# ComparativeGenomicsToolkit/cactus

Hardware: NVIDIA H100
Metric: BAR POA DP Gcells/sec and ends/sec at 1/2/4/8 H100 vs reference CPU BAR (higher is better)
Workload: dtype int32

## Files before the change

### cactus_b200/csrc/poa_kernel.cu

```cuda
#include <cuda_runtime.h>
#include <stdint.h>
#include "poa_graph.cuh"
#include "poa_cta.cuh"
#include "poa_kernel.cuh"

namespace barb200 {

#define FULL 0xffffffffu

struct KShared {
    Graph g; RowTables rt; DpState d;
    int job, msa_len_s, abort_s;
    __align__(256) int smat[5 * 8];
    int wF[2][2][32];
    int wM[2][4][32];
    RowRec rec[2];
    RowInfo ring_info[2];
};

__device__ __forceinline__ int4 ld4cg(const int *p) { return __ldcg(reinterpret_cast<const int4 *>(p)); }
__device__ __forceinline__ void st4(int *p, int a, int b, int c, int d) {
    asm volatile("st.global.v4.s32 [%0], {%1, %2, %3, %4};" ::"l"(p), "r"(a), "r"(b), "r"(c), "r"(d) : "memory");
}
__device__ __forceinline__ void sts4(unsigned a, int x, int y, int z, int w) {
    asm volatile("st.shared.v4.s32 [%0], {%1, %2, %3, %4};" ::"r"(a), "r"(x), "r"(y), "r"(z), "r"(w) : "memory");
}
__device__ __forceinline__ int4 lds4(unsigned a) {
    int4 v;
    asm volatile("ld.shared.v4.s32 {%0, %1, %2, %3}, [%4];" : "=r"(v.x), "=r"(v.y), "=r"(v.z), "=r"(v.w) : "r"(a) : "memory");
    return v;
}
__device__ __forceinline__ int lds1(unsigned a) {
    int v;
    asm volatile("ld.shared.s32 %0, [%1];" : "=r"(v) : "r"(a) : "memory");
    return v;
}
__device__ __forceinline__ int lds_const(unsigned a) {
    int v;
    asm("ld.shared.s32 %0, [%1];" : "=r"(v) : "r"(a));
    return v;
}
__device__ __forceinline__ int max3(int a, int b, int c) { return max(max(a, b), c); }
__device__ __forceinline__ void cp_async16(void *smem, const void *gmem) {
    asm volatile("cp.async.cg.shared.global [%0], [%1], 16;" ::"r"((unsigned)__cvta_generic_to_shared(smem)), "l"(gmem) : "memory");
}
__device__ __forceinline__ void cp_async_wait_all() { asm volatile("cp.async.wait_all;" ::: "memory"); }
__device__ __forceinline__ void store_pad(int *tp, int64_t cs, int NEG) {
#pragma unroll
    for (int c = 0; c < TB / CHUNK; ++c) st4(tp + c * cs, c < CPT / CHUNK ? NEG : 0, c < CPT / CHUNK ? NEG : 0, c < CPT / CHUNK ? NEG : 0, c < CPT / CHUNK ? NEG : 0);
}


template <bool MASKED>
__device__ __forceinline__ void row_pass1(int (&H)[CPT], int (&E1)[CPT], int (&E2)[CPT], unsigned mbase, const uint32_t (&qo)[4],
                                          int j0, int beg, int end, int NEG, int e1, int e2, int &agg1, int &agg2) {
#pragma unroll
    for (int e = 0; e < CPT; ++e) {
        const int s = lds_const(__byte_perm(qo[e >> 2], mbase, 0x7650 | (e & 3)));
        int h = __vimax3_s32(H[e] + s, E1[e], E2[e]);
        if (MASKED) {
            const bool inb = (unsigned)(j0 + e - beg) <= (unsigned)(end - beg);
            h = inb ? h : NEG; E1[e] = inb ? E1[e] : NEG; E2[e] = inb ? E2[e] : NEG;
        }
        H[e] = h;
    }
    int a1 = H[CPT - 1], a2 = H[CPT - 1];
#pragma unroll
    for (int e = CPT - 2; e >= 0; --e) { a1 = __viaddmax_s32(a1, e1, H[e]); a2 = __viaddmax_s32(a2, e2, H[e]); }
    agg1 = max(agg1, a1 + j0 * e1); agg2 = max(agg2, a2 + j0 * e2);
}

template <bool ROW0>
__device__ __forceinline__ void pred_chunk(int (&H)[CPT], int (&E1)[CPT], int (&E2)[CPT], int oc, int4 h4, int4 d4, int NEG) {
    const int h[CHUNK] = {h4.x, h4.y, h4.z, h4.w}, dv[CHUNK] = {d4.x, d4.y, d4.z, d4.w};
#pragma unroll
    for (int u = 0; u < CHUNK; ++u) {
        const int e = oc * CHUNK + u;
        const int c1 = dv[u] & 0xffff, c2 = (int)((unsigned)dv[u] >> 16);
        if (e + 1 < CPT) H[e + 1] = max(H[e + 1], h[u]);
        E1[e] = max(E1[e], ROW0 && c1 == E_NEG16 ? NEG : h[u] - c1); E2[e] = max(E2[e], ROW0 && c2 == E_NEG16 ? NEG : h[u] - c2);
    }
}

template <int MODE, int RING_NT>
__device__ __forceinline__ void row_pass2(int (&H)[CPT], int (&E1)[CPT], int (&E2)[CPT], int F1, int F2, int j0, int beg, int end, int NEG,
                                          int e1, int e2, int oe1, int oe2, int *tp, int64_t cs, unsigned rs, int &tmax) {
#pragma unroll
    for (int oc = 0; oc < CPT / CHUNK; ++oc) {
        int dd[CHUNK];
#pragma unroll
        for (int u = 0; u < CHUNK; ++u) {
            const int e = oc * CHUNK + u, hp = H[e];
            int h = __vimax3_s32(hp, F1, F2);
            F1 = __viaddmax_s32(F1, -e1, hp - oe1); F2 = __viaddmax_s32(F2, -e2, hp - oe2);
            int x1 = __viaddmax_s32(E1[e], -e1, h - oe1);
            int x2 = __viaddmax_s32(E2[e], -e2, h - oe2);
            if (MODE == 1) {
                const bool inb = (unsigned)(j0 + e - beg) <= (unsigned)(end - beg);
                h = inb ? h : NEG; x1 = inb ? x1 : NEG; x2 = inb ? x2 : NEG;
            } else if (MODE == 2) {
                const bool inb = j0 + e <= end;
                h = inb ? h : NEG; x1 = inb ? x1 : NEG; x2 = inb ? x2 : NEG;
            }
            H[e] = h; E1[e] = x1; E2[e] = x2;
            dd[u] = __byte_perm(h - x1, h - x2, 0x5410);
            tmax = max(tmax, h);
        }
        st4(tp + oc * cs, H[oc * CHUNK], H[oc * CHUNK + 1], H[oc * CHUNK + 2], H[oc * CHUNK + 3]);
        st4(tp + (CPT / CHUNK + oc) * cs, dd[0], dd[1], dd[2], dd[3]);
        if (RING_NT) {
            sts4(rs + oc * RING_NT * 16, H[oc * CHUNK], H[oc * CHUNK + 1], H[oc * CHUNK + 2], H[oc * CHUNK + 3]);
            sts4(rs + (CPT / CHUNK + oc) * RING_NT * 16, dd[0], dd[1], dd[2], dd[3]);
        }
    }
}

template <bool MASKED>
__device__ __forceinline__ void row_argmax(const int (&H)[CPT], int v, int j0, int beg, int end, int &tl, int &tr) {
    unsigned m = 0;
#pragma unroll
    for (int e = 0; e < CPT; ++e) m |= H[e] == v ? 1u << e : 0u;
    if (MASKED) {
        const int lo = max(beg - j0, 0), hi = min(end - j0, CPT - 1);
        m &= (2u << hi) - (1u << lo);
    }
    if (m) { tl = j0 + __ffs(m) - 1; tr = j0 + 31 - __clz(m); }
}

template <int NT>
__device__ long long dp_sweep(KShared &S, const BatchArgs &A, const uint8_t *__restrict__ qg, int L, uint4 *qsm, unsigned ring) {
    constexpr int RING_NT = poa_ring_bytes(NT) ? NT : 0;
    constexpr unsigned SLOT = NT * TB * sizeof(int), RCS = NT * 16;
    const int tid = threadIdx.x, lane = tid & 31, warp = tid >> 5, nwarps = NT >> 5;
    const unsigned my_ring = ring + tid * 16;
    const PoaParams &P = A.P;
    uint8_t *const sb = A.slots + (int64_t)blockIdx.x * A.lay.slot_bytes;
    const RowRec *const rec_tab = reinterpret_cast<const RowRec *>(sb + A.lay.o_row_rec);
    const int *const pre_row = reinterpret_cast<const int *>(sb + A.lay.o_pre_row);
    RowInfo *const info = reinterpret_cast<RowInfo *>(sb + A.lay.o_row_info);
    int64_t *const row_off = reinterpret_cast<int64_t *>(sb + A.lay.o_row_off);
    int *const planes = A.planes + (int64_t)blockIdx.x * A.lay.plane_cap;
    const int64_t plane_cap = A.lay.plane_cap;
    const int node_n = S.g.node_n, R = node_n - 1;
    const int NEG = P.inf_min, e1 = P.e1, e2 = P.e2, oe1 = P.o1 + P.e1, oe2 = P.o2 + P.e2;
    const int w = P.wb + (int)(P.wf * L);
    const int pn_shift = reference_lane_count(P, L, node_n) == 16 ? 4 : 3;
    static_assert(CPT == 16, "shifts below assume 16 columns per thread");
    const int j0 = tid * CPT;

    uint32_t qo[4] = {0u, 0u, 0u, 0u};
#pragma unroll
    for (int e = 0; e < CPT; ++e) {
        const int j = j0 + e;
        const uint32_t c = (j >= 1 && j <= L) ? qg[j - 1] : 5u;
        qo[e >> 2] |= (4u * c) << ((e & 3) * 8);
    }
    qsm[tid] = make_uint4(qo[0], qo[1], qo[2], qo[3]);
    const unsigned smat_s = (unsigned)__cvta_generic_to_shared(S.smat);

    int H[CPT], E1[CPT], E2[CPT];
    bool prev_active;
    int prev_beg = 0, prev_end, prev_left = 0, prev_right = 0;
    int cur_blk = 0, cells = 0;

    {
        const int dd = L - rec_tab[0].rd;
        prev_end = min(L, max(0, dd) + w);
        const int nT = prev_end / CPT + 1, nTs = row_blocks(0, prev_end);
        if ((int64_t)nTs * TB > plane_cap) return -1;
        prev_active = tid < nT;
        int D[CPT];
#pragma unroll
        for (int e = 0; e < CPT; ++e) {
            const int j = j0 + e;
            if (j == 0) { H[e] = 0; E1[e] = -oe1; E2[e] = -oe2; D[e] = oe1 | (oe2 << 16); }
            else if (j <= prev_end) { H[e] = max(-P.o1 - e1 * j, -P.o2 - e2 * j); E1[e] = NEG; E2[e] = NEG; D[e] = E_NEG16 | (E_NEG16 << 16); }
            else { H[e] = E1[e] = E2[e] = NEG; D[e] = 0; }
        }
        if (tid < nTs) {
            int *tp = planes + chunk_index(nTs, tid, 0);
            const int64_t cs = chunk_index(nTs, 0, 1);
#pragma unroll
            for (int oc = 0; oc < CPT / CHUNK; ++oc) {
                st4(tp + oc * cs, H[oc * CHUNK], H[oc * CHUNK + 1], H[oc * CHUNK + 2], H[oc * CHUNK + 3]);
                st4(tp + (CPT / CHUNK + oc) * cs, D[oc * CHUNK], D[oc * CHUNK + 1], D[oc * CHUNK + 2], D[oc * CHUNK + 3]);
            }
        }
        if (RING_NT) {
#pragma unroll
            for (int oc = 0; oc < CPT / CHUNK; ++oc) {
                sts4(my_ring + oc * RCS, H[oc * CHUNK], H[oc * CHUNK + 1], H[oc * CHUNK + 2], H[oc * CHUNK + 3]);
                sts4(my_ring + (CPT / CHUNK + oc) * RCS, D[oc * CHUNK], D[oc * CHUNK + 1], D[oc * CHUNK + 2], D[oc * CHUNK + 3]);
            }
        }
        if (lane == 31) S.wM[0][3][warp] = H[CPT - 1];
        if (tid == 0) {
            RowInfo ri; ri.beg = 0; ri.end = prev_end; ri.left = 0; ri.right = 0; info[0] = ri; row_off[0] = 0;
            if (RING_NT) S.ring_info[0] = ri;
        }
        cur_blk = nTs; cells = prev_end + 1;
        if (tid == 0) { cp_async16(&S.rec[1], rec_tab + (R > 1 ? 1 : 0)); cp_async_wait_all(); }
    }
    __syncthreads();

    for (int r = 1; r < R; ++r) {
        const int par = r & 1;
        const RowRec rec = S.rec[par];
        if (tid == 0 && r + 1 < R) cp_async16(&S.rec[par ^ 1], rec_tab + r + 1);
        const int b = rec.base_npre & 0xff, npre = rec.base_npre >> 8;
        const int dd = L - rec.rd;
        int maxL = node_n, maxR = 0, min_pre_beg = 0x7fffffff;
        bool has_prev = false;
        if (npre == 1 && rec.pre0 == r - 1) {
            maxL = min(node_n, prev_left + 1); maxR = prev_right + 1; min_pre_beg = prev_beg; has_prev = true;
        } else {
#pragma unroll 1
            for (int k = 0; k < npre; ++k) {
                const int p = k == 0 ? rec.pre0 : pre_row[rec.pre_off + k];
                int pl, pr, pb;
                if (p == r - 1) { pl = prev_left; pr = prev_right; pb = prev_beg; has_prev = true; }
                else if (RING_NT && p == r - 2) { const RowInfo pi = S.ring_info[par]; pl = pi.left; pr = pi.right; pb = pi.beg; }
                else { const RowInfo pi = info[p]; pl = pi.left; pr = pi.right; pb = pi.beg; }
                maxL = min(maxL, pl + 1); maxR = max(maxR, pr + 1); min_pre_beg = min(min_pre_beg, pb);
            }
        }
        const bool only_prev = npre == 1 && has_prev;
        int beg = max(0, min(maxL, dd) - w);
        const int end = min(L, max(maxR, dd) + w);
        if ((beg >> pn_shift) < (min_pre_beg >> pn_shift)) beg = min_pre_beg;
        const int t0 = beg >> 4, nT = (end >> 4) - t0 + 1, tt = tid - t0;
        const int nTs = row_blocks(beg, end), tts = tid - row_t0(beg);
        if ((int64_t)(cur_blk + nTs) * TB > plane_cap) return -1;
        const bool active = tt >= 0 && tt < nT;
        const int wmode = __any_sync(FULL, active && j0 < beg) ? 1 : __any_sync(FULL, active && j0 + CPT - 1 > end) ? 2 : 0;
        const uint32_t qadd = 0x01010101u * (32u * b);

        int hl = __shfl_up_sync(FULL, prev_active ? H[CPT - 1] : NEG, 1);
        if (lane == 0) hl = warp > 0 ? S.wM[par ^ 1][3][warp - 1] : NEG;

        const int id1 = NEG + beg * e1 + P.o1, id2 = NEG + beg * e2 + P.o2;
        int agg1 = id1, agg2 = id2;
        if (active) {
            if (has_prev && prev_active) {
#pragma unroll
                for (int e = CPT - 1; e >= 1; --e) H[e] = H[e - 1];
                H[0] = hl;
            } else {
#pragma unroll
                for (int e = 0; e < CPT; ++e) { H[e] = NEG; E1[e] = NEG; E2[e] = NEG; }
                if (has_prev) H[0] = hl;
            }
#pragma unroll 1
            for (int k = only_prev ? npre : 0; k < npre; ++k) {
                const int p = k == 0 ? rec.pre0 : pre_row[rec.pre_off + k];
                if (p == r - 1) continue;
                if (RING_NT && p == r - 2) {
                    const RowInfo pi = S.ring_info[par];
                    const int pt0 = pi.beg >> 4, pnT = (pi.end >> 4) - pt0 + 1, ptt = tid - pt0;
                    const unsigned rs = my_ring + par * SLOT;
                    if (ptt >= 0 && ptt < pnT) {
                        if (p == 0) {
#pragma unroll
                            for (int oc = 0; oc < CPT / CHUNK; ++oc) pred_chunk<true>(H, E1, E2, oc, lds4(rs + oc * RCS), lds4(rs + (CPT / CHUNK + oc) * RCS), NEG);
                        } else {
#pragma unroll
                            for (int oc = 0; oc < CPT / CHUNK; ++oc) pred_chunk<false>(H, E1, E2, oc, lds4(rs + oc * RCS), lds4(rs + (CPT / CHUNK + oc) * RCS), NEG);
                        }
                    }
                    if (ptt >= 1 && ptt <= pnT) H[0] = max(H[0], lds1(rs + (CPT / CHUNK - 1) * RCS - 4));
                    continue;
                }
                const RowInfo pi = info[p];
                const int pt0 = pi.beg >> 4, pnT = (pi.end >> 4) - pt0 + 1, ptt = tid - pt0, pnTs = row_blocks(pi.beg, pi.end);
                const int *Hp = planes + row_off[p] + chunk_index(pnTs, tid - row_t0(pi.beg), 0);
                const int64_t pcs = chunk_index(pnTs, 0, 1);
                if (ptt >= 0 && ptt < pnT) {
#pragma unroll
                    for (int oc = 0; oc < CPT / CHUNK; ++oc) pred_chunk<true>(H, E1, E2, oc, ld4cg(Hp + oc * pcs), ld4cg(Hp + (CPT / CHUNK + oc) * pcs), NEG);
                }
                if (ptt >= 1 && ptt <= pnT) H[0] = max(H[0], __ldcg(Hp - CHUNK + (CPT / CHUNK - 1) * pcs + CHUNK - 1));
            }
            const uint4 q4 = qsm[tid];
            const uint32_t qo[4] = {q4.x + qadd, q4.y + qadd, q4.z + qadd, q4.w + qadd};
            if (wmode != 1) row_pass1<false>(H, E1, E2, smat_s, qo, j0, beg, end, NEG, e1, e2, agg1, agg2);
            else row_pass1<true>(H, E1, E2, smat_s, qo, j0, beg, end, NEG, e1, e2, agg1, agg2);
        }
        int inc1 = agg1, inc2 = agg2;
#pragma unroll
        for (int off = 1; off < 32; off <<= 1) {
            const int n1 = __shfl_up_sync(FULL, inc1, off), n2 = __shfl_up_sync(FULL, inc2, off);
            if (lane >= off) { inc1 = max(inc1, n1); inc2 = max(inc2, n2); }
        }
        int ex1 = __shfl_up_sync(FULL, inc1, 1), ex2 = __shfl_up_sync(FULL, inc2, 1);
        if (lane == 0) { ex1 = id1; ex2 = id2; }
        if (lane == 31) { S.wF[par][0][warp] = inc1; S.wF[par][1][warp] = inc2; }
        __syncthreads();
        int P1, P2;
        {
            const int wv1 = lane < warp ? S.wF[par][0][lane] : id1, wv2 = lane < warp ? S.wF[par][1][lane] : id2;
            P1 = max(__reduce_max_sync(FULL, wv1), ex1); P2 = max(__reduce_max_sync(FULL, wv2), ex2);
        }
        int tmax = INT32_MIN;
        {
            int *tp = planes + (int64_t)cur_blk * TB + chunk_index(nTs, tts, 0);
            const int64_t cs = chunk_index(nTs, 0, 1);
            const unsigned rs = my_ring + par * SLOT;
            if (active) {
                const int F1 = P1 - P.o1 - j0 * e1, F2 = P2 - P.o2 - j0 * e2;
                if (wmode == 0) row_pass2<0, RING_NT>(H, E1, E2, F1, F2, j0, beg, end, NEG, e1, e2, oe1, oe2, tp, cs, rs, tmax);
                else if (wmode == 2) row_pass2<2, RING_NT>(H, E1, E2, F1, F2, j0, beg, end, NEG, e1, e2, oe1, oe2, tp, cs, rs, tmax);
                else row_pass2<1, RING_NT>(H, E1, E2, F1, F2, j0, beg, end, NEG, e1, e2, oe1, oe2, tp, cs, rs, tmax);
            } else if ((unsigned)tts < (unsigned)nTs) store_pad(tp, cs, NEG);
        }
        {
            const int wmax = __reduce_max_sync(FULL, tmax);
            int tleft = 0x7fffffff, tright = -1;
            if (active && tmax == wmax) {
                if (wmode == 0) row_argmax<false>(H, wmax, j0, beg, end, tleft, tright); else row_argmax<true>(H, wmax, j0, beg, end, tleft, tright);
            }
            const int wl = __reduce_min_sync(FULL, tleft), wr = __reduce_max_sync(FULL, tright);
            if (lane == 0) { S.wM[par][0][warp] = wmax; S.wM[par][1][warp] = wl; S.wM[par][2][warp] = wr; }
            if (lane == 31) S.wM[par][3][warp] = active ? H[CPT - 1] : NEG;
        }
        if (tid == 0) cp_async_wait_all();
        __syncthreads();
        {
            const int v = lane < nwarps ? S.wM[par][0][lane] : INT32_MIN;
            const int bmax = __reduce_max_sync(FULL, v);
            const int l = (lane < nwarps && v == bmax) ? S.wM[par][1][lane] : 0x7fffffff;
            const int rr = (lane < nwarps && v == bmax) ? S.wM[par][2][lane] : -1;
            prev_left = __reduce_min_sync(FULL, l); prev_right = __reduce_max_sync(FULL, rr);
        }
        prev_beg = beg; prev_end = end; prev_active = active;
        if (tid == 0) {
            RowInfo ri; ri.beg = beg; ri.end = end; ri.left = prev_left; ri.right = prev_right; info[r] = ri; row_off[r] = (int64_t)cur_blk * TB;
            if (RING_NT) S.ring_info[par] = ri;
        }
        cur_blk += nTs; cells += end - beg + 1;
    }
    __syncthreads();
    return cells;
}

#define PHASE_TICK(ph) do { if (A.phase_clk && threadIdx.x == 0) { unsigned long long _n = clock64(); A.phase_clk[(size_t)blockIdx.x * PH_N + (ph)] += _n - t_last; t_last = _n; } } while (0)

template <int NT>
__device__ __forceinline__ void poa_msa_body(const BatchArgs &A) {
    extern __shared__ __align__(16) unsigned char dyn_smem[];
    __shared__ KShared S;
    __shared__ uint4 qsm[NT];
    const int tid = threadIdx.x;
    int *ws = &S.wF[0][0][0];
    if (tid == 0) { const int slot = blockIdx.x; slot_views(A.lay, A.slots + (int64_t)slot * A.lay.slot_bytes, A.planes + (int64_t)slot * A.lay.plane_cap, S.g, S.rt, S.d); }
    for (int k = tid; k < 40; k += blockDim.x) S.smat[k] = (k & 7) < 5 ? A.P.mat[(k >> 3) * 5 + (k & 7)] : 0;
    unsigned long long t_last = A.phase_clk ? clock64() : 0ULL, t_start = t_last;
    __syncthreads();

    while (true) {
        if (tid == 0) {
            const int k = atomicAdd(A.next_job, 1);
            int j = -1;
            if (k < A.n_jobs) j = A.job_base + k;
            S.job = j;
        }
        __syncthreads();
        const int job = S.job;
        if (job < 0) break;
        const JobDesc jd = A.jobs[job];
        const int K = jd.n_seq;
        const int *lens = A.lens + jd.len_off;
        const int64_t *soff = A.soff + jd.len_off;
        const uint8_t *seqs = A.seqs + jd.seq_off;
        if (tid == 0) { graph_reset(S.g, K); S.abort_s = 0; }
        __syncthreads();
        const int *const order = A.order + jd.len_off;
        if (tid == 0 && A.gt_status[job]) S.g.err = JOB_ERR_GT_CAP;
        __syncthreads();
        long long cells = 0;
        for (int a = 0; a < K && !S.g.err; ++a) {
            const int read = order[a], L = lens[read];
            const uint8_t *q = seqs + soff[read];
            if (a == 0) {
                if (A.serial_phases) { if (tid == 0) graph_add_first_sequence(S.g, q, L, read); }
                else cta_add_first_sequence(S.g, q, L, read);
                PHASE_TICK(PH_FUSE);
            } else {
                long long c = -2;
                if (L + 1 <= CPT * (int)blockDim.x) c = dp_sweep<NT>(S, A, q, L, qsm, (unsigned)__cvta_generic_to_shared(dyn_smem));
                if (c < 0) { if (tid == 0) S.g.err = c == -2 ? JOB_ERR_QUERY_LEN : JOB_ERR_PLANE_CAP; c = 0; }
                cells += c;
                __syncthreads();
                PHASE_TICK(PH_DP);
                if (A.serial_phases) { if (tid == 0 && !S.g.err) { dp_best_cell(S.g, S.rt, S.d, A.P, L); dp_backtrack(S.g, S.rt, S.d, A.P, q, L); } }
                else if (tid < 32 && !S.g.err) warp_backtrack(S.g, S.rt, S.d, A.P, S.smat, q, L);
                PHASE_TICK(PH_BACKTRACK);
                __syncthreads();
                if (A.serial_phases) { if (tid == 0 && !S.g.err) graph_fuse_alignment(S.g, q, S.d.cigar, S.d.n_cigar, read); }
                else if (!S.g.err) cta_fuse_alignment(S.g, q, L, S.d.cigar, S.d.n_cigar, read, ws, dyn_smem, A.scratch_bytes);
                PHASE_TICK(PH_FUSE);
            }
            __syncthreads();
            if (S.g.err) break;
            if (A.serial_phases) { if (tid == 0) graph_topo_sort_serial(S.g, S.rt); __syncthreads(); }
            else cta_topo_sort(S.g, S.rt, dyn_smem, A.scratch_bytes, ws, A.bfs_order == 0);
            PHASE_TICK(PH_TOPO);
            if (S.g.err) break;
        }
        __syncthreads();
        if (!S.g.err) {
            if (A.serial_phases) { if (tid == 0) S.msa_len_s = graph_msa_rank(S.g); __syncthreads(); }
            else cta_msa_rank(S.g, dyn_smem, A.scratch_bytes, ws, &S.msa_len_s);
            if (tid == 0 && !S.g.err && S.msa_len_s > jd.msa_stride) S.g.err = JOB_ERR_MSA_CAP;
        }
        __syncthreads();
        if (!S.g.err) {
            const int ml = S.msa_len_s;
            uint8_t *msa = A.msa + jd.msa_off;
            for (int64_t i = tid; i < (int64_t)K * ml; i += blockDim.x) msa[(i / ml) * jd.msa_stride + (i % ml)] = GAP_CODE;
            __syncthreads();
            for (int v = 2 + tid; v < S.g.node_n; v += blockDim.x) graph_msa_fill_node(S.g, v, msa, jd.msa_stride);
        }
        __syncthreads();
        if (tid == 0) { A.status[job] = S.g.err; A.msa_len[job] = S.g.err ? 0 : S.msa_len_s; A.cells[job] = cells; }
        PHASE_TICK(PH_MSA);
        __syncthreads();
    }
    if (A.phase_clk && tid == 0) A.phase_clk[(size_t)blockIdx.x * PH_N + PH_TOTAL] += clock64() - t_start;
}

extern "C" __global__ void __launch_bounds__(32, 16) poa_msa_kernel_t32(const BatchArgs A) { poa_msa_body<32>(A); }
extern "C" __global__ void __launch_bounds__(64, 8) poa_msa_kernel_t64(const BatchArgs A) { poa_msa_body<64>(A); }
#ifndef BARB200_T128_MINB
#define BARB200_T128_MINB 4
#endif
extern "C" __global__ void __launch_bounds__(128, BARB200_T128_MINB) poa_msa_kernel_t128(const BatchArgs A) { poa_msa_body<128>(A); }
extern "C" __global__ void __launch_bounds__(256, 2) poa_msa_kernel_t256(const BatchArgs A) { poa_msa_body<256>(A); }
extern "C" __global__ void __launch_bounds__(640, 1) poa_msa_kernel_t640(const BatchArgs A) { poa_msa_body<640>(A); }
extern "C" __global__ void __launch_bounds__(1024, 1) poa_msa_kernel_t1024(const BatchArgs A) { poa_msa_body<1024>(A); }

}
```

### cactus_b200/csrc/poa_types.h

```cpp
#pragma once
#include <stdint.h>

#if defined(__CUDACC__)
#define HD __host__ __device__ __forceinline__
#else
#define HD inline
#endif

#if defined(__CUDA_ARCH__)
#define GT_THREADS(tid, T) for (int tid = (int)threadIdx.x, _gt_once = 1; _gt_once; _gt_once = 0)
#define GT_SYNC() __syncthreads()
#else
#define GT_THREADS(tid, T) for (int tid = 0; tid < (T); ++tid)
#define GT_SYNC() ((void)0)
#endif

namespace barb200 {

constexpr int SRC_ID = 0;
constexpr int SINK_ID = 1;
constexpr int GAP_CODE = 5;

constexpr int OP_M = 0x1, OP_E1 = 0x2, OP_E2 = 0x4, OP_E = 0x6, OP_F1 = 0x8, OP_F2 = 0x10, OP_F = 0x18, OP_ALL = 0x1f;
constexpr int CMATCH = 0, CINS = 1, CDEL = 2;

enum JobStatus : int {
    JOB_OK = 0,
    JOB_ERR_NODE_CAP = 1,
    JOB_ERR_EDGE_CAP = 2,
    JOB_ERR_PLANE_CAP = 3,
    JOB_ERR_CIGAR_CAP = 4,
    JOB_ERR_MSA_CAP = 5,
    JOB_ERR_TOPO = 6,
    JOB_ERR_BACKTRACK = 7,
    JOB_ERR_ALIGNED_CAP = 8,
    JOB_ERR_QUERY_LEN = 9,
    JOB_ERR_GT_CAP = 10
};

struct PoaParams {
    int mat[25];
    int o1, e1, o2, e2;
    int wb; float wf;
    int max_mat, min_mis;
    int inf_min;
};

struct JobDesc {
    int n_seq;
    int64_t seq_off;
    int64_t len_off;
    int64_t msa_off;
    int msa_stride;
    int progressive;
};

struct Graph {
    int node_n, node_cap;
    int W;
    int in_used, in_pool, out_used, out_pool;
    int err;
    uint8_t *base;
    uint8_t *aln_n;
    int *aln_id;
    int *in_off, *in_n, *in_cap;
    int *out_off, *out_n, *out_cap;
    int *in_id, *in_w;
    int *out_id, *out_w;
    uint64_t *out_rid;
    int *index_to_node, *node_to_index;
    int *remain;
    int *msa_rank;
    int *tmp0, *tmp1;
};

struct alignas(16) RowRec {
    int base_npre;
    int rd;
    int pre_off;
    int pre0;
};
struct RowTables {
    RowRec *rec;
    int *pre_row;
};

struct alignas(16) RowInfo {
    int beg, end;
    int left, right;
};

constexpr int CPT = 16;
constexpr int E_NEG16 = 0xffff;
struct DpState {
    int *planes; int64_t plane_cap;
    int64_t *row_off;
    RowInfo *info;
    uint64_t *cigar; int n_cigar, cigar_cap;
    int best_i, best_j, best_score;
    int *fc;
    int fc_cap, fc_row, fc_hi;
};

constexpr int TB = 2 * CPT;
constexpr int CHUNK = 4;
HD int row_t0(int beg) { return (beg / CPT) & ~1; }
HD int row_blocks(int beg, int end) { return ((end / CPT - row_t0(beg)) | 1) + 1; }
HD int64_t chunk_index(int nblk, int b, int c) { return ((int64_t)c * nblk + b) * CHUNK; }
HD int64_t plane_index(int beg, int end, int plane, int j) {
    return chunk_index(row_blocks(beg, end), j / CPT - row_t0(beg), plane * (CPT / CHUNK) + j % CPT / CHUNK) + j % CHUNK;
}
HD int64_t row_ints(int beg, int end) { return (int64_t)TB * row_blocks(beg, end); }
HD int e_decode(int h, int code, int inf_min) { return code == E_NEG16 ? inf_min : h - code; }
HD int e_encode(int h, int e) { const int d = h - e; return (d >= 0 && d < E_NEG16) ? d : E_NEG16; }

HD int imax(int a, int b) { return a > b ? a : b; }
HD int imin(int a, int b) { return a < b ? a : b; }

inline PoaParams poa_params(const int mat[25], int o1, int e1, int o2, int e2, int wb, float wf) {
    PoaParams P;
    P.o1 = o1; P.e1 = e1; P.o2 = o2; P.e2 = e2; P.wb = wb; P.wf = wf;
    P.max_mat = 0; P.min_mis = 0;
    for (int i = 0; i < 25; ++i) { P.mat[i] = mat[i]; P.max_mat = imax(P.max_mat, mat[i]); P.min_mis = imax(P.min_mis, -mat[i]); }
    P.inf_min = imax(imax(INT32_MIN + P.min_mis, INT32_MIN + o1 + e1), INT32_MIN + o2 + e2) + 512 * imax(e1, e2);
    return P;
}

}
```

Baseline: 264.3.

## Merge row max/argmax into first barrier phase, dropping second per-row syncthreads

Moves the per-warp row max and argmax reduction, plus the warp boundary H publish, from after pass2 to before the first __syncthreads, computing them on pass1 H values. The boundary H value is then fixed up with the F prefix by lane 0 after the barrier. This removes one block-wide barrier per DP row. The risk is that max/argmax are now taken on pre-F H values, which could be incorrect where the F gap term raises H, and the left-boundary fixup adds a shared-memory dependence between warps.

```diff
diff --git a/cactus_b200/csrc/poa_kernel.cu b/cactus_b200/csrc/poa_kernel.cu
--- a/cactus_b200/csrc/poa_kernel.cu
+++ b/cactus_b200/csrc/poa_kernel.cu
@@ -84,7 +84,7 @@
 
 template <int MODE, int RING_NT>
 __device__ __forceinline__ void row_pass2(int (&H)[CPT], int (&E1)[CPT], int (&E2)[CPT], int F1, int F2, int j0, int beg, int end, int NEG,
-                                          int e1, int e2, int oe1, int oe2, int *tp, int64_t cs, unsigned rs, int &tmax) {
+                                          int e1, int e2, int oe1, int oe2, int *tp, int64_t cs, unsigned rs) {
 #pragma unroll
     for (int oc = 0; oc < CPT / CHUNK; ++oc) {
         int dd[CHUNK];
@@ -104,7 +104,6 @@
             }
             H[e] = h; E1[e] = x1; E2[e] = x2;
             dd[u] = __byte_perm(h - x1, h - x2, 0x5410);
-            tmax = max(tmax, h);
         }
         st4(tp + oc * cs, H[oc * CHUNK], H[oc * CHUNK + 1], H[oc * CHUNK + 2], H[oc * CHUNK + 3]);
         st4(tp + (CPT / CHUNK + oc) * cs, dd[0], dd[1], dd[2], dd[3]);
@@ -113,6 +112,17 @@
             sts4(rs + (CPT / CHUNK + oc) * RING_NT * 16, dd[0], dd[1], dd[2], dd[3]);
         }
     }
+}
+
+template <bool MASK_RIGHT>
+__device__ __forceinline__ int row_prefmax(const int (&H)[CPT], int j0, int end, int NEG) {
+    int h[CPT];
+#pragma unroll
+    for (int e = 0; e < CPT; ++e) h[e] = !MASK_RIGHT || j0 + e <= end ? H[e] : NEG;
+    int m = __vimax3_s32(h[0], h[1], h[2]);
+#pragma unroll
+    for (int e = 3; e + 1 < CPT; e += 2) m = __vimax3_s32(m, h[e], h[e + 1]);
+    return max(m, h[CPT - 1]);
 }
 
 template <bool MASKED>
@@ -240,6 +250,7 @@
 
         const int id1 = NEG + beg * e1 + P.o1, id2 = NEG + beg * e2 + P.o2;
         int agg1 = id1, agg2 = id2;
+        int tmax = INT32_MIN;
         if (active) {
             if (has_prev && prev_active) {
 #pragma unroll
@@ -284,46 +295,49 @@
             const uint32_t qo[4] = {q4.x + qadd, q4.y + qadd, q4.z + qadd, q4.w + qadd};
             if (wmode != 1) row_pass1<false>(H, E1, E2, smat_s, qo, j0, beg, end, NEG, e1, e2, agg1, agg2);
             else row_pass1<true>(H, E1, E2, smat_s, qo, j0, beg, end, NEG, e1, e2, agg1, agg2);
+            tmax = row_prefmax<false>(H, j0, end, NEG);
+            if (wmode == 2) tmax = row_prefmax<true>(H, j0, end, NEG);
+        }
+        {
+            const int wmax = __reduce_max_sync(FULL, tmax);
+            int tleft = 0x7fffffff, tright = -1;
+            if (active && tmax == wmax) {
+                if (wmode == 0) row_argmax<false>(H, wmax, j0, beg, end, tleft, tright); else row_argmax<true>(H, wmax, j0, beg, end, tleft, tright);
+            }
+            const int wl = __reduce_min_sync(FULL, tleft), wr = __reduce_max_sync(FULL, tright);
+            if (lane == 0) { S.wM[par][0][warp] = wmax; S.wM[par][1][warp] = wl; S.wM[par][2][warp] = wr; }
+            if (lane == 31) S.wM[par][3][warp] = H[CPT - 1];
         }
         int inc1 = agg1, inc2 = agg2;
 #pragma unroll
         for (int off = 1; off < 32; off <<= 1) {
-            const int n1 = __shfl_up_sync(FULL, inc1, off), n2 = __shfl_up_sync(FULL, inc2, off);
-            if (lane >= off) { inc1 = max(inc1, n1); inc2 = max(inc2, n2); }
+            inc1 = max(inc1, __shfl_up_sync(FULL, inc1, off)); inc2 = max(inc2, __shfl_up_sync(FULL, inc2, off));
         }
         int ex1 = __shfl_up_sync(FULL, inc1, 1), ex2 = __shfl_up_sync(FULL, inc2, 1);
         if (lane == 0) { ex1 = id1; ex2 = id2; }
         if (lane == 31) { S.wF[par][0][warp] = inc1; S.wF[par][1][warp] = inc2; }
+        if (tid == 0) cp_async_wait_all();
         __syncthreads();
         int P1, P2;
         {
             const int wv1 = lane < warp ? S.wF[par][0][lane] : id1, wv2 = lane < warp ? S.wF[par][1][lane] : id2;
             P1 = max(__reduce_max_sync(FULL, wv1), ex1); P2 = max(__reduce_max_sync(FULL, wv2), ex2);
         }
-        int tmax = INT32_MIN;
+        if (lane == 0 && warp > 0) {
+            int &hw = S.wM[par][3][warp - 1];
+            hw = sweep_left_h(hw, P1 - P.o1 - j0 * e1, P2 - P.o2 - j0 * e2, e1, e2, tt >= 1 && tt <= nT && j0 - 1 <= end, NEG);
+        }
         {
             int *tp = planes + (int64_t)cur_blk * TB + chunk_index(nTs, tts, 0);
             const int64_t cs = chunk_index(nTs, 0, 1);
             const unsigned rs = my_ring + par * SLOT;
             if (active) {
                 const int F1 = P1 - P.o1 - j0 * e1, F2 = P2 - P.o2 - j0 * e2;
-                if (wmode == 0) row_pass2<0, RING_NT>(H, E1, E2, F1, F2, j0, beg, end, NEG, e1, e2, oe1, oe2, tp, cs, rs, tmax);
-                else if (wmode == 2) row_pass2<2, RING_NT>(H, E1, E2, F1, F2, j0, beg, end, NEG, e1, e2, oe1, oe2, tp, cs, rs, tmax);
-                else row_pass2<1, RING_NT>(H, E1, E2, F1, F2, j0, beg, end, NEG, e1, e2, oe1, oe2, tp, cs, rs, tmax);
+                if (wmode == 0) row_pass2<0, RING_NT>(H, E1, E2, F1, F2, j0, beg, end, NEG, e1, e2, oe1, oe2, tp, cs, rs);
+                else if (wmode == 2) row_pass2<2, RING_NT>(H, E1, E2, F1, F2, j0, beg, end, NEG, e1, e2, oe1, oe2, tp, cs, rs);
+                else row_pass2<1, RING_NT>(H, E1, E2, F1, F2, j0, beg, end, NEG, e1, e2, oe1, oe2, tp, cs, rs);
             } else if ((unsigned)tts < (unsigned)nTs) store_pad(tp, cs, NEG);
         }
-        {
-            const int wmax = __reduce_max_sync(FULL, tmax);
-            int tleft = 0x7fffffff, tright = -1;
-            if (active && tmax == wmax) {
-                if (wmode == 0) row_argmax<false>(H, wmax, j0, beg, end, tleft, tright); else row_argmax<true>(H, wmax, j0, beg, end, tleft, tright);
-            }
-            const int wl = __reduce_min_sync(FULL, tleft), wr = __reduce_max_sync(FULL, tright);
-            if (lane == 0) { S.wM[par][0][warp] = wmax; S.wM[par][1][warp] = wl; S.wM[par][2][warp] = wr; }
-            if (lane == 31) S.wM[par][3][warp] = active ? H[CPT - 1] : NEG;
-        }
-        if (tid == 0) cp_async_wait_all();
-        __syncthreads();
         {
             const int v = lane < nwarps ? S.wM[par][0][lane] : INT32_MIN;
             const int bmax = __reduce_max_sync(FULL, v);
diff --git a/cactus_b200/csrc/poa_types.h b/cactus_b200/csrc/poa_types.h
--- a/cactus_b200/csrc/poa_types.h
+++ b/cactus_b200/csrc/poa_types.h
@@ -117,6 +117,10 @@
 HD int imax(int a, int b) { return a > b ? a : b; }
 HD int imin(int a, int b) { return a < b ? a : b; }
 
+HD int sweep_left_h(int hp, int f1, int f2, int e1, int e2, bool live, int inf_min) {
+    return live ? imax(imax(hp, f1 + e1), f2 + e2) : inf_min;
+}
+
 inline PoaParams poa_params(const int mat[25], int o1, int e1, int o2, int e2, int wb, float wf) {
     PoaParams P;
     P.o1 = o1; P.e1 = e1; P.o2 = o2; P.e2 = e2; P.wb = wb; P.wf = wf;
```

After: 267.9, median of 6. 1.01x the previous value.
